# miguelmartin75/txt2vid

Measured on AMD Instinct MI355X. Metric: TGANv2 GAN train throughput (G+D steps x global batch), 16x64x64 videos/sec, higher is better.
Workload: dtype f32; 1 GPU; BASELINE configs[1]: unconditional TGANv2 16x64x64x1, per-GPU batch 32, fp32, RSGAN + GP 0.5, Adam 2e-4 (0.5,0.999), 1 D + 1 G step, subsample_input pyramid 8/16/32/64; global_batch=32, per_gpu_batch=32, parallelism=dp1

## Files before the change

### include/t2v_hip.h

```cpp
#ifndef T2V_HIP_H
#define T2V_HIP_H

#include <stdint.h>

#ifdef __cplusplus
extern "C" {
#endif

#define T2V_OK 0
#define T2V_EINVAL (-1)
#define T2V_ELAUNCH (-2)

#define T2V_MAX_TAPS 27

typedef struct {
    int32_t N, Cin, D, H, W, Cout;
    int32_t ntaps;
    int8_t dz[T2V_MAX_TAPS], dy[T2V_MAX_TAPS], dx[T2V_MAX_TAPS];
    int8_t pad_[3];
} t2v_conv_geom;

#define T2V_MAX_GROUPS 8
typedef struct {
    const float* x;
// ... 238 lines not shown

int t2v_copy2d(const float* src, int64_t src_ld, float* dst, int64_t dst_ld, int64_t rows, int64_t cols, void* stream);
int t2v_cast_bf16(const void* src, void* dst, int64_t n, int dir, void* stream);
int t2v_permute01(const float* x, float* y, int64_t A, int64_t B, int64_t inner, void* stream);
int t2v_permute12(const float* x, float* y, int64_t A, int64_t B, int64_t C, int64_t inner, void* stream);
int t2v_subsample_frames(float* x, float* y, int64_t b, int64_t T, int64_t inner, int64_t bo, int64_t To, int bt,
                         int adjoint, const int32_t* bt_dev , void* stream);
int t2v_pyramid_scatter(const float* g, float* gx, int B, int C, int T, int64_t HW, int Bo, int To, int sb, int st,
                        int bt, void* stream);


int t2v_scalar_combine(const void* const* ptrs, const float* weights, int n, float* out, void* stream);
int t2v_gather_rows(const float* x, const int32_t* perm, float* out, int64_t rows, int64_t cols, int inverse, void* stream);


typedef struct t2v_poolbox_job {
    const float* in;
    const float* mask;
    float* out;
    const float* bias;
    int32_t NC, D, H, W;
    int32_t tmode, relu;
    float scale;
    int32_t C;
} t2v_poolbox_job;
int t2v_pool_boxsum(const t2v_poolbox_job* jobs, int njobs, void* stream);
int t2v_pool_unbox(const t2v_poolbox_job* jobs, int njobs, void* stream);
int64_t t2v_pool_conv_fwd_ws_floats(const t2v_conv_group* groups, int ngroups, int Cin, int Cout);
int t2v_pool_conv_fwd(const t2v_conv_group* groups, int ngroups, int Cin, int Cout, const float* wp, const float* bias, float* ws,
                      int flags, void* stream);
// ... 59 lines not shown
```

### txt2vid_amd/_lib.py

```python
import ctypes as C
import os

_HERE = os.path.dirname(os.path.abspath(__file__))
LIB_PATH = os.environ.get('T2V_LIB') or os.path.join(_HERE, 'csrc', 'libt2v_hip.so')

MAX_TAPS = 27


class ConvGeom(C.Structure):
    _fields_ = [('N', C.c_int32), ('Cin', C.c_int32), ('D', C.c_int32), ('H', C.c_int32), ('W', C.c_int32),
                ('Cout', C.c_int32), ('ntaps', C.c_int32),
                ('dz', C.c_int8 * MAX_TAPS), ('dy', C.c_int8 * MAX_TAPS), ('dx', C.c_int8 * MAX_TAPS),
                ('pad_', C.c_int8 * 3)]


class ConvGroup(C.Structure):
    _fields_ = [('x', C.c_void_p), ('y', C.c_void_p), ('mask', C.c_void_p), ('N', C.c_int32), ('D', C.c_int32), ('H', C.c_int32), ('W', C.c_int32),
                ('ntaps', C.c_int32), ('dstride', C.c_int32), ('ydstride', C.c_int32), ('yoff', C.c_int32), ('Dy', C.c_int32),
                ('dz', C.c_int8 * MAX_TAPS), ('dy', C.c_int8 * MAX_TAPS), ('dx', C.c_int8 * MAX_TAPS), ('widx', C.c_int8 * MAX_TAPS)]


class AdamJob(C.Structure):
    _fields_ = [('p', C.c_void_p), ('g', C.c_void_p), ('m', C.c_void_p), ('v', C.c_void_p), ('n', C.c_int64)]

# ... 154 lines not shown
    't2v_adam_multi': [_P, _I, _F, _F, _F, _F, _F, _F, _F, _P, _P],
    't2v_sgd_multi': [_P, _I, _F, _F, _F, _I, _P],
    't2v_adam_tick': [_P, _F, _F, _P],
    't2v_ema_multi': [_P, _I, _F, _F, _P, _F, _P],
    't2v_ema_tick': [_P, _P],
    't2v_swap_multi': [_P, _I, _P],
    't2v_pyramid_gather': [_P, _P, _I, _I, _I, _I, _I, _I, _I, _I, _I, _I, _I, _I, _P, _P],
    't2v_copy2d': [_P, _L, _P, _L, _L, _L, _P],
    't2v_cast_bf16': [_P, _P, _L, _I, _P],
    't2v_permute01': [_P, _P, _L, _L, _L, _P],
    't2v_permute12': [_P, _P, _L, _L, _L, _L, _P],
    't2v_subsample_frames': [_P, _P, _L, _L, _L, _L, _L, _I, _I, _P, _P],
    't2v_pyramid_scatter': [_P, _P, _I, _I, _I, _L, _I, _I, _I, _I, _I, _P],
    't2v_scalar_combine': [_P, C.POINTER(C.c_float), _I, _P, _P],
    't2v_gather_rows': [_P, _P, _P, _L, _L, _I, _P],
    't2v_pool_boxsum': [_P, _I, _P],
    't2v_pool_unbox': [_P, _I, _P],
    't2v_pool_conv_fwd_ws_floats': [_P, _I, _I, _I],
    't2v_pool_conv_fwd': [_P, _I, _I, _I, _P, _P, _P, _I, _P],
    't2v_pool_conv_dgrad': [_P, _I, _I, _I, _P, _P],
    't2v_pool_conv_dgrad_splits': [_P, _I, _I, _I],
    't2v_pool_conv_wgrad_slab_floats': [_P, _I, _I, _I, _I, _I],
    't2v_pool_conv_wgrad': [_P, _I, _I, _I, _I, _P, _P, _P, _I, _P],
    't2v_pool_conv_wgrad_partial': [_P, _I, _I, _I, _I, _P, _I, _I, _P, _P],
    't2v_wgrad_swap': [_P, _P, _I, _I, _I, _I, _P],
    't2v_pool_conv_plan': [_I, _P, _I, _I, _I, _I3],
    't2v_synth_clips': [_P, _I, _L, _I, _I, _I, _I3, _P, _P, _P, _P],
    't2v_clip_gather': [_P, _L, _P, _I, _I, _I, _I, _I, _P, _P, _P, _P],
    't2v_tseed_fwd_bn': [_P, _P, _P, _P, _P, _P, _P, _P, _P, _P, _P, _I, _I, _I, _I, _I, _F, _F, _I, _P],
    't2v_tseed_fwd_tanh': [_P, _P, _P, _P, _P, _I, _I, _I, _I, _P],
# ... 39 lines not shown
```

### txt2vid_amd/csrc/conv.hip

```cpp
#include <hip/hip_runtime.h>
#include <stdint.h>
#include "../../include/t2v_hip.h"

typedef float f32x16 __attribute__((ext_vector_type(16)));

#ifdef T2V_STAMPS
__device__ unsigned long long* g_stamps = nullptr;
__device__ unsigned int g_stamps_cap = 0;
extern "C" int t2v_stamps_set(void* buf, unsigned int cap_records) {
    if (hipMemcpyToSymbol(HIP_SYMBOL(g_stamps), &buf, sizeof(buf)) != hipSuccess) return -1;
    if (hipMemcpyToSymbol(HIP_SYMBOL(g_stamps_cap), &cap_records, sizeof(cap_records)) != hipSuccess) return -1;
    return 0;
}
__device__ __forceinline__ unsigned long long stamp_now() {
    unsigned long long t;
    __builtin_amdgcn_sched_barrier(0);
    asm volatile("s_memtime %0\n\ts_waitcnt lgkmcnt(0)" : "=s"(t) :: "memory");
    __builtin_amdgcn_sched_barrier(0);
    return t;
}
#define STAMP(v) const unsigned long long v = stamp_now()
#define STAMP_ACC(acc, a, b) acc += (b) - (a)
#else
#define STAMP(v)
// ... 1081 lines not shown
    __shared__ __attribute__((aligned(16))) float Bs[(DB ? 2 : 1) * 3 * BKT * BN];

    const int tid = threadIdx.x;
    const int lane = tid & 63, wave = tid >> 6;
    const int l31 = lane & 31, hi = lane >> 5;
    const int wco = wave % WAVES_CO, wm = wave / WAVES_CO;

    const int tile = xcd_remap((int)blockIdx.x, (int)gridDim.x);
    int gi = 0;
#pragma unroll
    for (int k = 1; k < T2V_MAX_GROUPS; ++k)
        if (k < tab.n && tile >= tab.tile_start[k]) gi = k;
    const t2v_conv_group& gd = tab.g[gi];
    const int tm = gd.dstride;
    const int Dn = tm ? gd.D / 2 : 1, Hn = gd.H / 2, Wn = gd.W / 2;
    const int Hp = gd.H + 1, Wp = gd.W + 2, Dp = tm ? gd.D + 1 : 1;
    const int Vp = Dp * Hp * Wp;
    const int HWn = Hn * Wn, DHWn = Dn * HWn;
    const int M = gd.N * DHWn;
    const int m0 = (tile - tab.tile_start[gi]) * BM, co0 = blockIdx.y * BN;
    const int ntaps = gd.ntaps;
    const int nrow = ntaps / 3;

    const int lane_r = lane < nrow ? lane : 0, lane_t = lane < ntaps ? lane : 0;
    const int tab_roff = ((tm ? gd.dz[lane_r * 3] + 1 : 0) * Hp + gd.dy[lane_r * 3] + 1) * Wp * 4;
    const int tab_widx = gd.widx[lane_t];
    const __amdgpu_buffer_rsrc_t rx = __builtin_amdgcn_make_buffer_rsrc((void*)gd.x, 0, (int)((uint32_t)(gd.N * Vp) * (uint32_t)Cin * 4u), 0x00020000);
    const __amdgpu_buffer_rsrc_t rw = __builtin_amdgcn_make_buffer_rsrc((void*)wp, 0, -1, 0x00020000);

    const int ma_l = tid % BM, ka_l = tid / BM;
    uint32_t xbase = 0;
// ... 213 lines not shown
    const int wco = wave % WAVES_CO, wm = wave / WAVES_CO;

    const int tile = xcd_remap((int)blockIdx.x, (int)gridDim.x);
    int gi = 0;
#pragma unroll
    for (int k = 1; k < T2V_MAX_GROUPS; ++k)
        if (k < tab.n && tile >= tab.tile_start[k]) gi = k;
    const t2v_conv_group& gd = tab.g[gi];
    const int tm = gd.dstride;
    const int nct = (int)gridDim.y >> 2;
    const int pair = (int)blockIdx.y / nct, ct = pair >> 1, cy = pair & 1;
    if (tm == 0 && ct) return;
    const int co0 = ((int)blockIdx.y - pair * nct) * BN;
    const int Dn = tm ? gd.D / 2 : 1, Hn = gd.H / 2, Wn = gd.W / 2;
    const int Dq = tm ? Dn + 1 : 1, Hq = Hn + 1, Wq = Wn + 1;
    const int HWn = Hn * Wn, Vn = Dn * HWn;
    const int HWq = Hq * Wq, Vq = Dq * HWq;
    const int De = (tm && ct) ? Dn : Dq, He = cy ? Hn : Hq;
    const int HWe = He * Wq, Ve = De * HWe;
    const int M = gd.N * Ve;
    const int m0 = (tile - tab.tile_start[gi]) * BM;
    if (m0 >= M) return;
    const int ndz = (tm && ct == 0) ? 2 : 1, ndy = cy == 0 ? 2 : 1;
    const int nrow = ndz * ndy;
    const int lane_t = lane < 27 ? lane : 0;
    const int tab_widx = gd.widx[lane_t];
    const __amdgpu_buffer_rsrc_t rx = __builtin_amdgcn_make_buffer_rsrc((void*)gd.x, 0, (int)((uint32_t)(gd.N * Vn) * (uint32_t)K * 4u), 0x00020000);
    const __amdgpu_buffer_rsrc_t rw = __builtin_amdgcn_make_buffer_rsrc((void*)wp, 0, -1, 0x00020000);

    const int ma_l = tid % BM, ka_l = tid / BM;
    const int hk = tid % BKT;
    const bool halo_thread = tid < BKT;
// ... 217 lines not shown
                const float xo = a_own[krow * AP], xl = a_left[krow * AP];
                acc0 = __builtin_amdgcn_mfma_f32_32x32x2f32(b0[krow * BN], xo, acc0, 0, 0, 0);
                acc1 = __builtin_amdgcn_mfma_f32_32x32x2f32(b1[krow * BN], xo, acc1, 0, 0, 0);
                acc0 = __builtin_amdgcn_mfma_f32_32x32x2f32(b2[krow * BN], xl, acc0, 0, 0, 0);
            }
        }
        __builtin_amdgcn_s_setprio(0);
        __syncthreads();
    }
    }
    const int m = m0 + wm * WM + l31;
    if (m < M) {
        const int n = m / Ve, spe = m - n * Ve;
        const int at = spe / HWe, r2 = spe - at * HWe;
        const int a = r2 / Wq, b = r2 - a * Wq;
        const int sp = (at * Hq + a) * Wq + b;
        constexpr bool row_ok = true;
        const bool ok1 = b < Wn;
        const size_t plane = (size_t)gd.N * C * Vq;
        float* p0 = gd.y + ((size_t)blockIdx.z * 8 + (size_t)((ct * 2 + cy) * 2 + 0)) * plane + (size_t)n * C * Vq + sp;
        float* p1 = p0 + plane;
#pragma unroll
        for (int r = 0; r < 16; ++r) {
            const int co = co0 + wco * WCO + (r & 3) + 8 * (r >> 2) + 4 * hi;
            if (co < C) {
                if (row_ok) p0[(size_t)co * Vq] = acc0[r];
                if (ok1) p1[(size_t)co * Vq] = acc1[r];
            }
        }
    }
}
// ... 2208 lines not shown
#pragma unroll
        for (int k = 1; k < T2V_MAX_GROUPS; ++k)
            if (k < tab.n && q >= tab.chunk_start[k]) gi = k;
        const t2v_conv_group& gd = tab.g[gi];
        g_i = gi;
        g_begin = tab.chunk_start[gi];
        g_end = tab.chunk_start[gi + 1];
        g_tm = gd.dstride;
        const int Dn = g_tm ? gd.D / 2 : 1;
        gHn = gd.H / 2; gWn = gd.W / 2; gHWn = gHn * gWn; gVn = Dn * gHWn;
        gM = gd.N * gVn;
        g_pow2 = ((Dn & (Dn - 1)) | (gHn & (gHn - 1)) | (gWn & (gWn - 1))) == 0;
        g_lw = __builtin_ctz(gWn);
        g_lhw = g_lw + __builtin_ctz(gHn);
        g_lv = g_lhw + __builtin_ctz(Dn);
        gHp = gd.H + 1; gWp = gd.W + 2;
        gVp = (g_tm ? gd.D + 1 : 1) * gHp * gWp;
        g_x = __builtin_amdgcn_make_buffer_rsrc((void*)gd.x, 0, (int)((uint32_t)(gd.N * gVp) * (uint32_t)Cin * 4u), 0x00020000);
        g_y = __builtin_amdgcn_make_buffer_rsrc((void*)gd.y, 0, (int)((uint32_t)gM * (uint32_t)Cout * 4u), 0x00020000);
    };

    auto load_chunk = [&](int q) {
        if (q >= g_end || g_i < 0) enter_group(q);
        const int m = (q - g_begin) * WG_BK + ml;
        const bool mv = m < gM;
        int n, sp, e, i, j;
        if (g_pow2) {
            n = m >> g_lv;
            sp = m & (gVn - 1);
            e = sp >> g_lhw;
            i = (sp >> g_lw) & (gHn - 1);
// ... 550 lines not shown
    WGroupTable tab;
    WgradPlan p;
    if (!build_wtable(groups, ngroups, Cin, Cout, kD, kH, kW, false, tab, p)) return T2V_EINVAL;
    float dummy;
    return wgrad_impl(groups, ngroups, Cin, Cout, kD, kH, kW, nullptr, want_bias ? &dummy : nullptr, slab, flags, stream, out_src);
}
struct PoolPlan { int S; long tiles; bool vecb; };
static bool pool_member_ok(const t2v_conv_group& g, bool need_ptrs) {
    if (need_ptrs && (!g.x || !g.y)) return false;
    if (g.N < 1 || g.H < 2 || g.W < 2 || (g.H & 1) || (g.W & 1)) return false;
    if (g.dstride == 0) return g.D == 1;
    if (g.dstride != 1 && g.dstride != 2) return false;
    return g.D >= 2 && !(g.D & 1);
}
static inline long pool_rows(const t2v_conv_group& g) { return (long)g.N * (g.dstride ? g.D / 2 : 1) * (g.H / 2) * (g.W / 2); }
static inline long pool_padded(const t2v_conv_group& g) { return (long)(g.dstride ? g.D + 1 : 1) * (g.H + 1) * (g.W + 2); }
static inline long pool_grid(const t2v_conv_group& g) { return (long)(g.dstride ? g.D / 2 + 1 : 1) * (g.H / 2 + 1) * (g.W / 2 + 1); }

static bool build_pool_fwd(const t2v_conv_group* groups, int ngroups, int Cin, int Cout, bool need_ptrs, GroupTable& tab, PoolPlan& p) {
    if (!groups || ngroups < 1 || ngroups > T2V_MAX_GROUPS || Cin < 32 || (Cin % 32) || Cout < 4 || (Cout % 4)) return false;
    long mt = 0, ot = 0;
    int max_rows = 1;
    tab.n = ngroups;
    for (int i = 0; i < ngroups; ++i) {
        const t2v_conv_group& g = groups[i];
        if (!pool_member_ok(g, need_ptrs)) return false;
        if ((long)g.N * pool_padded(g) * Cin >= (1L << 29) || pool_rows(g) * Cout >= (1L << 31)) return false;
        if (g.ntaps != 9 && g.ntaps != 27) return false;
        if (g.dstride == 0 && g.ntaps != 9) return false;
        for (int r = 0; r < g.ntaps / 3; ++r)
            for (int d = 0; d < 3; ++d) {
// ... 69 lines not shown
        long blocks = (tab.out_start[ngroups] + 255) / 256;
        if (blocks > 2048) blocks = 2048;
        ProfScope prof_r(4, 0.0, s, Mtot, Cin, Cout, taps, ngroups, p.S);
        T2V_LAUNCH_PROF(splitk_reduce_kernel, dim3((unsigned)blocks), dim3(256), 0, s, tab, ws, bias, p.S, Cout, flags);
    }
    return launch_status();
}

static bool build_pool_dgrad(const t2v_conv_group* groups, int ngroups, int K, int C, bool need_ptrs, GroupTable& tab, PoolPlan& p) {
    if (!groups || ngroups < 1 || ngroups > T2V_MAX_GROUPS || K < 32 || (K % 32) || C < 4 || (C % 4)) return false;
    long mt = 0;
    tab.n = ngroups;
    for (int i = 0; i < ngroups; ++i) {
        const t2v_conv_group& g = groups[i];
        if (!pool_member_ok(g, need_ptrs)) return false;
        if (pool_rows(g) * K >= (1L << 29) || (long)g.N * pool_grid(g) * C * 8 >= (1L << 31)) return false;
        for (int f = 0; f < 27; ++f) {
            const bool live = g.dstride != 0 || (f / 9) == 1;
            if (live && (g.widx[f] < 0 || g.widx[f] >= T2V_MAX_TAPS)) return false;
        }
        tab.g[i] = g;
        tab.tile_start[i] = (int32_t)mt;
        tab.out_start[i] = 0;
        mt += ((long)g.N * pool_grid(g) + 63) / 64;
    }
    for (int i = ngroups; i <= T2V_MAX_GROUPS; ++i) { tab.tile_start[i] = (int32_t)mt; tab.out_start[i] = 0; }
    p.tiles = mt * 4 * ((C + 63) / 64);
    p.vecb = (C % 4) == 0;
    long S = 1;
    const long ncb = K / 32;
    static const long split_below = env_long("T2V_POOL_DGRAD_SPLIT_BELOW", 576);
// ... 487 lines not shown
```

### txt2vid_amd/csrc/pointwise.hip

```cpp
#include <hip/hip_runtime.h>
#include <stdint.h>
#include "../../include/t2v_hip.h"

#define T2V_LAUNCH(...) do { (void)hipGetLastError(); hipLaunchKernelGGL(__VA_ARGS__); } while (0)

static inline int launch_status() {
    hipError_t e = hipGetLastError();
    return e == hipSuccess ? T2V_OK : -(int)e - 1000;
}
static inline unsigned nblocks(long n, int per = 256) {
    long b = (n + per - 1) / per;
    if (b > 2048) b = 2048;
    if (b < 1) b = 1;
    return (unsigned)b;
}
#define GRID_STRIDE(i, n) for (long i = (long)blockIdx.x * blockDim.x + threadIdx.x; i < (n); i += (long)gridDim.x * blockDim.x)
#define S_(stream) ((hipStream_t)(stream))

__device__ __forceinline__ float wave_sum(float v) {
#pragma unroll
    for (int o = 32; o > 0; o >>= 1) v += __shfl_xor(v, o, 64);
    return v;
}
__device__ __forceinline__ float wave_max(float v) {
// ... 2650 lines not shown
    T2V_LAUNCH(gather_rows_k, dim3(nblocks(rows * cols)), dim3(256), 0, S_(st), x, perm, out, (long)rows, (long)cols, inverse);
    return launch_status();
}

extern "C" const char* t2v_version(void) { return "t2v_hip 0.1 (gfx950, fp32 MFMA)"; }

struct PoolBoxBatch { t2v_poolbox_job j[POOL_MT]; int begin[POOL_MT + 1]; int n; };

__device__ __forceinline__ uint32_t small_div(uint32_t m, uint32_t d, float rcp) {
    int q = (int)((float)m * rcp);
    const int r = (int)m - q * (int)d;
    q += (r >= (int)d) ? 1 : 0;
    q -= (r < 0) ? 1 : 0;
    return (uint32_t)q;
}
__global__ __launch_bounds__(256) void pool_boxsum_k(const PoolBoxBatch tb) {
    int ji = 0;
#pragma unroll
    for (int k = 1; k < POOL_MT; ++k)
        if (k < tb.n && (int)blockIdx.x >= tb.begin[k]) ji = k;
    const t2v_poolbox_job& q = tb.j[ji];
    const int D = q.D, H = q.H, W = q.W, tm = q.tmode;
    const uint32_t Dp = tm ? D + 1 : 1, Hp = H + 1, Wp = W + 2, Wp2 = Wp / 2;
    const uint32_t n2 = (uint32_t)q.NC * Dp * Hp * Wp2;
    const uint32_t base = (uint32_t)((int)blockIdx.x - tb.begin[ji]) * POOL_CHUNK;
    const uint32_t b_r0 = base / Wp2, b_x = base - b_r0 * Wp2;
    const uint32_t b_r1 = b_r0 / Hp, b_y = b_r0 - b_r1 * Hp;
    const uint32_t b_nc = b_r1 / Dp, b_f = b_r1 - b_nc * Dp;
    const float rW = 1.0f / (float)Wp2, rH = 1.0f / (float)Hp, rD = 1.0f / (float)Dp;
    const float* __restrict__ x = q.in;
    const float* __restrict__ mk = q.mask;
    const float floor_ = q.relu ? 0.f : -__builtin_inff();
    const float scale = q.scale;
    const int nf = tm == 1 ? 2 : 1;
    float2* __restrict__ out2 = reinterpret_cast<float2*>(q.out);
#pragma unroll
    for (int it = 0; it < POOL_CHUNK / 256; ++it) {
        const uint32_t t = it * 256 + threadIdx.x;
// ... 22 lines not shown
                if (y0 && c1) v01 = mk[o + 1] > 0.f ? v01 : 0.f;
                if (y0 && c2) v02 = mk[o + 2] > 0.f ? v02 : 0.f;
                if (y1 && c0) v10 = mk[o + W] > 0.f ? v10 : 0.f;
                if (y1 && c1) v11 = mk[o + W + 1] > 0.f ? v11 : 0.f;
                if (y1 && c2) v12 = mk[o + W + 2] > 0.f ? v12 : 0.f;
            }
            v00 = fmaxf(v00, floor_); v01 = fmaxf(v01, floor_); v02 = fmaxf(v02, floor_);
            v10 = fmaxf(v10, floor_); v11 = fmaxf(v11, floor_); v12 = fmaxf(v12, floor_);
            a0 += (v00 + v01) + (v10 + v11);
            a1 += (v01 + v02) + (v11 + v12);
        }
        out2[base + t] = make_float2(a0 * scale, xp + 1 <= (uint32_t)W ? a1 * scale : 0.f);
    }
}

__global__ __launch_bounds__(256) void pool_unbox_k(const PoolBoxBatch tb) {
    int ji = 0;
#pragma unroll
    for (int k = 1; k < POOL_MT; ++k)
        if (k < tb.n && (int)blockIdx.x >= tb.begin[k]) ji = k;
    const t2v_poolbox_job& q = tb.j[ji];
    const uint32_t D = q.D, H = q.H, W = q.W, W2 = W / 2;
    const int tm = q.tmode;
    const uint32_t Dq = tm ? D / 2 + 1 : 1, Hq = H / 2 + 1, Wq = W / 2 + 1;
    const uint32_t n2 = (uint32_t)q.NC * D * H * W2;
    const uint32_t plane = (uint32_t)q.NC * Dq * Hq * Wq;
    const int sets = q.relu > 1 ? q.relu : 1;
    const uint32_t base = (uint32_t)((int)blockIdx.x - tb.begin[ji]) * POOL_CHUNK;
    const uint32_t b_r0 = base / W2, b_x = base - b_r0 * W2;
    const uint32_t b_r1 = b_r0 / H, b_y = b_r0 - b_r1 * H;
    const uint32_t b_nc = b_r1 / D, b_f = b_r1 - b_nc * D;
    const float rW = 1.0f / (float)W2, rH = 1.0f / (float)H, rD = 1.0f / (float)D;
    const float* __restrict__ pl = q.in;
    const float2* __restrict__ mk2 = reinterpret_cast<const float2*>(q.mask);
    float2* __restrict__ out2 = reinterpret_cast<float2*>(q.out);
    const int nf = tm == 1 ? 2 : 1;
#pragma unroll
    for (int it = 0; it < POOL_CHUNK / 256; ++it) {
        const uint32_t t = it * 256 + threadIdx.x;
// ... 16 lines not shown
                    const uint32_t o1 = o0 + plane;
                    for (int s_ = 0; s_ < sets; ++s_) {
                        const uint32_t so = (uint32_t)s_ * 8u * plane;
                        const float e0 = pl[o0 + so], e1 = pl[o0 + 1 + so], d1 = pl[o1 + so];
                        a0 += e0 + d1;
                        a1 += e1 + d1;
                    }
                }
            }
        }
        const float bv = q.bias ? q.bias[nc % (uint32_t)q.C] : 0.f;
        out2[base + t] = make_float2(m2.x > 0.f ? a0 * q.scale + bv : 0.f, m2.y > 0.f ? a1 * q.scale + bv : 0.f);
    }
}

static int poolbox_multi(const t2v_poolbox_job* jobs, int njobs, bool unbox, void* st) {
    if (!jobs || njobs < 1) return T2V_EINVAL;
    for (int at = 0; at < njobs; at += POOL_MT) {
        PoolBoxBatch tb;
        const int cnt = njobs - at < POOL_MT ? njobs - at : POOL_MT;
        long blocks = 0;
        for (int i = 0; i < cnt; ++i) {
            const t2v_poolbox_job& q = jobs[at + i];
            if (!q.in || !q.out || q.NC < 1 || q.D < 1 || q.H < 2 || q.W < 2 || (q.H & 1) || (q.W & 1) || q.tmode < 0 || q.tmode > 2) return T2V_EINVAL;
            if ((q.tmode == 0 && q.D != 1) || (q.tmode != 0 && (q.D < 2 || (q.D & 1)))) return T2V_EINVAL;
            if (q.bias && (!unbox || q.C < 1 || (q.NC % q.C) != 0)) return T2V_EINVAL;
            tb.j[i] = q;
            tb.begin[i] = (int)blocks;
            const long n = unbox ? (long)q.NC * q.D * q.H * q.W
                                 : (long)q.NC * (q.tmode ? q.D + 1 : 1) * (q.H + 1) * (q.W + 2);
            const long sets = unbox && q.relu > 1 ? q.relu : 1;
            if (n >= (1L << 31) || (unbox && 8 * sets * (long)q.NC * (q.tmode ? q.D / 2 + 1 : 1) * (q.H / 2 + 1) * (q.W / 2 + 1) >= (1L << 31)))
                return T2V_EINVAL;
            if (((uintptr_t)q.out & 7u) || (unbox && q.mask && ((uintptr_t)q.mask & 7u))) return T2V_EINVAL;
            blocks += (n / 2 + POOL_CHUNK - 1) / POOL_CHUNK;
        }
        for (int i = cnt; i <= POOL_MT; ++i) tb.begin[i] = (int)blocks;
        for (int i = cnt; i < POOL_MT; ++i) tb.j[i] = tb.j[0];
        tb.n = cnt;
        if (blocks > 0x7fffffffL) return T2V_EINVAL;
        if (unbox) T2V_LAUNCH(pool_unbox_k, dim3((unsigned)blocks), dim3(256), 0, S_(st), tb);
        else T2V_LAUNCH(pool_boxsum_k, dim3((unsigned)blocks), dim3(256), 0, S_(st), tb);
    }
    return launch_status();
}
extern "C" int t2v_pool_boxsum(const t2v_poolbox_job* jobs, int njobs, void* st) { return poolbox_multi(jobs, njobs, false, st); }
extern "C" int t2v_pool_unbox(const t2v_poolbox_job* jobs, int njobs, void* st) { return poolbox_multi(jobs, njobs, true, st); }

__global__ __launch_bounds__(256) void wgrad_swap_k(const float* __restrict__ src, float* __restrict__ dst, int Cout, int Cin, int T, int accum) {
    const long n = (long)Cout * Cin * T;
    GRID_STRIDE(i, n) {
        const int t = (int)(i % T); const long r = i / T;
        const int ci = (int)(r % Cin), co = (int)(r / Cin);
        const float v = src[((long)ci * Cout + co) * T + (T - 1 - t)];
        dst[i] = accum ? dst[i] + v : v;
    }
}
// ... 79 lines not shown
```

### txt2vid_amd/functional_pool.py

```python
import ctypes as C
import os

import torch
from torch.autograd import Function
from torch.autograd.function import once_differentiable

from ._lib import lib, check, ConvGroup, PoolBoxJob, WgradSrc, MAX_GROUPS
from ._ops import _stream, _p, _c

_DISABLED = os.environ.get('T2V_NO_POOLCONV') is not None
_NO_UPCONV = os.environ.get('T2V_NO_UPCONV') is not None


def _TF():
    from . import functional
    return functional


def pool_tmode(shape, stem):
    D, H, W = shape[2], shape[3], shape[4]
    if H < 2 or W < 2 or H % 2 or W % 2:
        return None
    if D == 1:
        return 0
# ... 3 lines not shown


def pool_scale(tmode):
    return 0.125 if tmode == 1 else 0.25


def pool_conv_ok(xs, w, stem):
    TF = _TF()
    if _DISABLED or TF.CONV_PRECISION != 'fp32' or not (1 <= len(xs) <= MAX_GROUPS) or w.dim() != 5 or tuple(w.shape[2:]) != (3, 3, 3):
        return False
    if w.shape[0] % 32 or w.shape[1] % 32 or not xs[0].is_cuda:
        return False
    return all(x.dim() == 5 and pool_tmode(x.shape, stem) is not None for x in xs)


def pooled_shape(shape, tmode):
    N, _, D, H, W = shape
    return (N, D // 2 if tmode else 1, H // 2, W // 2)



def _box_jobs(ins, masks, outs, shapes, tmodes, relu, scale=None, bias=None):
    arr = (PoolBoxJob * len(ins))()
    for a, t, sh, tm, i in zip(arr, ins, shapes, tmodes, range(len(ins))):
        a.in_, a.out = t.data_ptr(), outs[i].data_ptr()
        a.mask = masks[i].data_ptr() if masks is not None else None
        a.bias = bias.data_ptr() if bias is not None else None
        a.NC, a.D, a.H, a.W, a.C = sh[0] * sh[1], sh[2], sh[3], sh[4], sh[1]
        a.tmode, a.relu, a.scale = tm, int(relu), pool_scale(tm) if scale is None else scale
    return arr


def boxsum_raw(ins, tmodes, relu, masks=None, scale=None):
    ins = [_c(t) for t in ins]
    masks = [_c(m) for m in masks] if masks is not None else None
    shapes = [tuple(t.shape) for t in ins]
    outs = [torch.empty((sh[0], sh[1], sh[2] + 1 if tm else 1, sh[3] + 1, sh[4] + 2), device=t.device, dtype=torch.float32)
            for t, sh, tm in zip(ins, shapes, tmodes)]
    check(lib().t2v_pool_boxsum(_box_jobs(ins, masks, outs, shapes, tmodes, relu, scale), len(ins), _stream()), 't2v_pool_boxsum')
    return outs


def unbox_raw(planes, shapes, tmodes, masks=None, scale=None, bias=None):
    masks = [_c(m) for m in masks] if masks is not None else None
    outs = [torch.empty(tuple(sh), device=p.device, dtype=torch.float32) for p, sh in zip(planes, shapes)]
    sets = planes[0].shape[0] if planes[0].dim() == 7 else 1
    check(lib().t2v_pool_unbox(_box_jobs(planes, masks, outs, shapes, tmodes, sets, scale, bias), len(planes), _stream()), 't2v_pool_unbox')
    return outs


def _tap_union(tmodes, kD=3):
    TF = _TF()
# ... 54 lines not shown
    cout, cin = (w5.shape[1], w5.shape[0]) if transpose else (w5.shape[0], w5.shape[1])
    ts = _tap_union(tmodes, w5.shape[2])
    slot_of = {t: j for j, t in enumerate(ts.taps)}
    arr = (ConvGroup * len(gzs))()
    for a, g, sh, tm in zip(arr, gzs, shapes, tmodes):
        if tuple(g.shape) != (sh[0], cout) + pooled_shape(sh, tm)[1:]:
            raise ValueError('pooled gradient of shape %s for a member of shape %s' % (tuple(g.shape), tuple(sh)))
        a.x, a.y, a.mask = g.data_ptr(), None, None
        a.N, a.D, a.H, a.W = sh[0], sh[2], sh[3], sh[4]
        a.dstride, a.ntaps = tm, 27
        for f in range(27):
            a.widx[f] = slot_of.get(26 - f, -1) if ts.T == 27 else (slot_of.get(8 - (f - 9), -1) if 9 <= f < 18 else -1)
    S = int(lib().t2v_pool_conv_dgrad_splits(arr, len(gzs), cout, cin))
    if S < 1:
        raise RuntimeError('bad pooled data-gradient geometry')
    planes = [torch.empty((S, 8, sh[0], cin, sh[2] // 2 + 1 if tm else 1, sh[3] // 2 + 1, sh[4] // 2 + 1), device=g.device, dtype=torch.float32)
              for g, sh, tm in zip(gzs, shapes, tmodes)]
    for a, pl in zip(arr, planes):
        a.y = pl.data_ptr()
    wp = TF.packed_weight(w5, ts, 0 if transpose else 1)
    check(lib().t2v_pool_conv_dgrad(arr, len(gzs), cout, cin, _p(wp), _stream()), 't2v_pool_conv_dgrad')
    return planes


def _wgrad_table(rts, gzs, shapes, tmodes):
    arr = (ConvGroup * len(rts))()
    for a, x, g, sh, tm in zip(arr, rts, gzs, shapes, tmodes):
        a.x, a.y, a.mask = x.data_ptr(), g.data_ptr(), None
        a.N, a.D, a.H, a.W = sh[0], sh[2], sh[3], sh[4]
        a.dstride, a.ntaps = tm, 27 if tm else 9
    return arr
# ... 218 lines not shown
```

Baseline: 3008 videos/s.

## Pad pooled box-sum planes to 4-float pitch and add vectorized box/unbox kernels

Pads the innermost row extent of the box-sum and pooled data-gradient planes to a multiple of four floats, and updates the conv forward, dgrad and wgrad indexing plus the host allocations to use the new pitch. New box-sum and unbox kernels each handle four or eight outputs per thread with 128-bit buffer loads and stores. The old pair kernels stay as a fallback when widths or alignment do not fit. This is meant to cut memory-instruction count in the pooling stages, at the cost of slightly larger buffers and padded columns that must stay consistent across all consumers.

```diff
diff --git a/include/t2v_hip.h b/include/t2v_hip.h
--- a/include/t2v_hip.h
+++ b/include/t2v_hip.h
@@ -276,6 +276,8 @@
 int t2v_gather_rows(const float* x, const int32_t* perm, float* out, int64_t rows, int64_t cols, int inverse, void* stream);
 
 
+#define T2V_POOL_PITCH(n) (((n) + 3) & ~3)
+int t2v_pool_pitch(int n);
 typedef struct t2v_poolbox_job {
     const float* in;
     const float* mask;
diff --git a/txt2vid_amd/_lib.py b/txt2vid_amd/_lib.py
--- a/txt2vid_amd/_lib.py
+++ b/txt2vid_amd/_lib.py
@@ -192,6 +192,7 @@
     't2v_pyramid_scatter': [_P, _P, _I, _I, _I, _L, _I, _I, _I, _I, _I, _P],
     't2v_scalar_combine': [_P, C.POINTER(C.c_float), _I, _P, _P],
     't2v_gather_rows': [_P, _P, _P, _L, _L, _I, _P],
+    't2v_pool_pitch': [_I],
     't2v_pool_boxsum': [_P, _I, _P],
     't2v_pool_unbox': [_P, _I, _P],
     't2v_pool_conv_fwd_ws_floats': [_P, _I, _I, _I],
diff --git a/txt2vid_amd/csrc/conv.hip b/txt2vid_amd/csrc/conv.hip
--- a/txt2vid_amd/csrc/conv.hip
+++ b/txt2vid_amd/csrc/conv.hip
@@ -1119,7 +1119,7 @@
     const t2v_conv_group& gd = tab.g[gi];
     const int tm = gd.dstride;
     const int Dn = tm ? gd.D / 2 : 1, Hn = gd.H / 2, Wn = gd.W / 2;
-    const int Hp = gd.H + 1, Wp = gd.W + 2, Dp = tm ? gd.D + 1 : 1;
+    const int Hp = gd.H + 1, Wp = T2V_POOL_PITCH(gd.W + 2), Dp = tm ? gd.D + 1 : 1;
     const int Vp = Dp * Hp * Wp;
     const int HWn = Hn * Wn, DHWn = Dn * HWn;
     const int M = gd.N * DHWn;
@@ -1363,8 +1363,9 @@
     const int co0 = ((int)blockIdx.y - pair * nct) * BN;
     const int Dn = tm ? gd.D / 2 : 1, Hn = gd.H / 2, Wn = gd.W / 2;
     const int Dq = tm ? Dn + 1 : 1, Hq = Hn + 1, Wq = Wn + 1;
+    const int Pq = T2V_POOL_PITCH(Wq);
     const int HWn = Hn * Wn, Vn = Dn * HWn;
-    const int HWq = Hq * Wq, Vq = Dq * HWq;
+    const int Vq = Dq * Hq * Pq;
     const int De = (tm && ct) ? Dn : Dq, He = cy ? Hn : Hq;
     const int HWe = He * Wq, Ve = De * HWe;
     const int M = gd.N * Ve;
@@ -1612,7 +1613,7 @@
         const int n = m / Ve, spe = m - n * Ve;
         const int at = spe / HWe, r2 = spe - at * HWe;
         const int a = r2 / Wq, b = r2 - a * Wq;
-        const int sp = (at * Hq + a) * Wq + b;
+        const int sp = (at * Hq + a) * Pq + b;
         constexpr bool row_ok = true;
         const bool ok1 = b < Wn;
         const size_t plane = (size_t)gd.N * C * Vq;
@@ -3851,7 +3852,7 @@
         g_lw = __builtin_ctz(gWn);
         g_lhw = g_lw + __builtin_ctz(gHn);
         g_lv = g_lhw + __builtin_ctz(Dn);
-        gHp = gd.H + 1; gWp = gd.W + 2;
+        gHp = gd.H + 1; gWp = T2V_POOL_PITCH(gd.W + 2);
         gVp = (g_tm ? gd.D + 1 : 1) * gHp * gWp;
         g_x = __builtin_amdgcn_make_buffer_rsrc((void*)gd.x, 0, (int)((uint32_t)(gd.N * gVp) * (uint32_t)Cin * 4u), 0x00020000);
         g_y = __builtin_amdgcn_make_buffer_rsrc((void*)gd.y, 0, (int)((uint32_t)gM * (uint32_t)Cout * 4u), 0x00020000);
@@ -4432,7 +4433,8 @@
     return g.D >= 2 && !(g.D & 1);
 }
 static inline long pool_rows(const t2v_conv_group& g) { return (long)g.N * (g.dstride ? g.D / 2 : 1) * (g.H / 2) * (g.W / 2); }
-static inline long pool_padded(const t2v_conv_group& g) { return (long)(g.dstride ? g.D + 1 : 1) * (g.H + 1) * (g.W + 2); }
+static inline long pool_padded(const t2v_conv_group& g) { return (long)(g.dstride ? g.D + 1 : 1) * (g.H + 1) * T2V_POOL_PITCH(g.W + 2); }
+static inline long pool_plane(const t2v_conv_group& g) { return (long)(g.dstride ? g.D / 2 + 1 : 1) * (g.H / 2 + 1) * T2V_POOL_PITCH(g.W / 2 + 1); }
 static inline long pool_grid(const t2v_conv_group& g) { return (long)(g.dstride ? g.D / 2 + 1 : 1) * (g.H / 2 + 1) * (g.W / 2 + 1); }
 
 static bool build_pool_fwd(const t2v_conv_group* groups, int ngroups, int Cin, int Cout, bool need_ptrs, GroupTable& tab, PoolPlan& p) {
@@ -4532,7 +4534,7 @@
     for (int i = 0; i < ngroups; ++i) {
         const t2v_conv_group& g = groups[i];
         if (!pool_member_ok(g, need_ptrs)) return false;
-        if (pool_rows(g) * K >= (1L << 29) || (long)g.N * pool_grid(g) * C * 8 >= (1L << 31)) return false;
+        if (pool_rows(g) * K >= (1L << 29) || (long)g.N * pool_plane(g) * C * 8 >= (1L << 31)) return false;
         for (int f = 0; f < 27; ++f) {
             const bool live = g.dstride != 0 || (f / 9) == 1;
             if (live && (g.widx[f] < 0 || g.widx[f] >= T2V_MAX_TAPS)) return false;
diff --git a/txt2vid_amd/csrc/pointwise.hip b/txt2vid_amd/csrc/pointwise.hip
--- a/txt2vid_amd/csrc/pointwise.hip
+++ b/txt2vid_amd/csrc/pointwise.hip
@@ -2688,14 +2688,14 @@
     q -= (r < 0) ? 1 : 0;
     return (uint32_t)q;
 }
-__global__ __launch_bounds__(256) void pool_boxsum_k(const PoolBoxBatch tb) {
+__global__ __launch_bounds__(256) void pool_boxsum_pair_k(const PoolBoxBatch tb) {
     int ji = 0;
 #pragma unroll
     for (int k = 1; k < POOL_MT; ++k)
         if (k < tb.n && (int)blockIdx.x >= tb.begin[k]) ji = k;
     const t2v_poolbox_job& q = tb.j[ji];
     const int D = q.D, H = q.H, W = q.W, tm = q.tmode;
-    const uint32_t Dp = tm ? D + 1 : 1, Hp = H + 1, Wp = W + 2, Wp2 = Wp / 2;
+    const uint32_t Dp = tm ? D + 1 : 1, Hp = H + 1, Wp = T2V_POOL_PITCH(W + 2), Wp2 = Wp / 2;
     const uint32_t n2 = (uint32_t)q.NC * Dp * Hp * Wp2;
     const uint32_t base = (uint32_t)((int)blockIdx.x - tb.begin[ji]) * POOL_CHUNK;
     const uint32_t b_r0 = base / Wp2, b_x = base - b_r0 * Wp2;
@@ -2748,7 +2748,7 @@
     }
 }
 
-__global__ __launch_bounds__(256) void pool_unbox_k(const PoolBoxBatch tb) {
+__global__ __launch_bounds__(256) void pool_unbox_pair_k(const PoolBoxBatch tb) {
     int ji = 0;
 #pragma unroll
     for (int k = 1; k < POOL_MT; ++k)
@@ -2756,7 +2756,7 @@
     const t2v_poolbox_job& q = tb.j[ji];
     const uint32_t D = q.D, H = q.H, W = q.W, W2 = W / 2;
     const int tm = q.tmode;
-    const uint32_t Dq = tm ? D / 2 + 1 : 1, Hq = H / 2 + 1, Wq = W / 2 + 1;
+    const uint32_t Dq = tm ? D / 2 + 1 : 1, Hq = H / 2 + 1, Wq = T2V_POOL_PITCH(W / 2 + 1);
     const uint32_t n2 = (uint32_t)q.NC * D * H * W2;
     const uint32_t plane = (uint32_t)q.NC * Dq * Hq * Wq;
     const int sets = q.relu > 1 ? q.relu : 1;
@@ -2803,12 +2803,164 @@
     }
 }
 
+#define POOL_WIDE 256
+typedef uint32_t pool_u32x4 __attribute__((ext_vector_type(4)));
+__device__ __forceinline__ __amdgpu_buffer_rsrc_t pool_rsrc(const void* p, uint32_t bytes) {
+    return __builtin_amdgcn_make_buffer_rsrc(const_cast<void*>(p), 0, (int)bytes, 0x00020000);
+}
+__device__ __forceinline__ float4 pool_ld4(__amdgpu_buffer_rsrc_t r, uint32_t off, bool ok, uint32_t bytes) {
+    return __builtin_bit_cast(float4, __builtin_amdgcn_raw_buffer_load_b128(r, ok ? off : bytes, 0, 0));
+}
+__device__ __forceinline__ float pool_ld1(__amdgpu_buffer_rsrc_t r, uint32_t off, bool ok, uint32_t bytes) {
+    return __builtin_bit_cast(float, __builtin_amdgcn_raw_buffer_load_b32(r, ok ? off : bytes, 0, 0));
+}
+__device__ __forceinline__ void pool_st4(__amdgpu_buffer_rsrc_t r, uint32_t off, float4 v) {
+    __builtin_amdgcn_raw_buffer_store_b128(__builtin_bit_cast(pool_u32x4, v), r, off, 0, 0);
+}
+
+__global__ __launch_bounds__(256) void pool_boxsum_k(const PoolBoxBatch tb) {
+    int ji = 0;
+#pragma unroll
+    for (int k = 1; k < POOL_MT; ++k)
+        if (k < tb.n && (int)blockIdx.x >= tb.begin[k]) ji = k;
+    const t2v_poolbox_job& q = tb.j[ji];
+    const int D = q.D, H = q.H, W = q.W, tm = q.tmode;
+    const uint32_t Dp = tm ? D + 1 : 1, Hp = H + 1, P4 = T2V_POOL_PITCH(W + 2) / 4;
+    const uint32_t n4 = (uint32_t)q.NC * Dp * Hp * P4;
+    const uint32_t base = (uint32_t)((int)blockIdx.x - tb.begin[ji]) * POOL_WIDE;
+    const uint32_t t = threadIdx.x;
+    if (base + t >= n4) return;
+    const uint32_t b_r0 = base / P4, b_x = base - b_r0 * P4;
+    const uint32_t b_r1 = b_r0 / Hp, b_y = b_r0 - b_r1 * Hp;
+    const uint32_t b_nc = b_r1 / Dp, b_f = b_r1 - b_nc * Dp;
+    const float rW = 1.0f / (float)P4, rH = 1.0f / (float)Hp, rD = 1.0f / (float)Dp;
+    const uint32_t ix = b_x + t, q1 = small_div(ix, P4, rW), xq = (ix - q1 * P4) * 4;
+    const uint32_t iy = b_y + q1, q2 = small_div(iy, Hp, rH), yp = iy - q2 * Hp;
+    const uint32_t if_ = b_f + q2, q3 = small_div(if_, Dp, rD), fp = if_ - q3 * Dp;
+    const uint32_t nc = b_nc + q3;
+    const uint32_t in_bytes = (uint32_t)q.NC * D * H * W * 4u;
+    const __amdgpu_buffer_rsrc_t rin = pool_rsrc(q.in, in_bytes);
+    const __amdgpu_buffer_rsrc_t rmk = pool_rsrc(q.mask ? q.mask : q.in, in_bytes);
+    const __amdgpu_buffer_rsrc_t rout = pool_rsrc(q.out, n4 * 16u);
+    const bool has_mask = q.mask != nullptr;
+    const float floor_ = q.relu ? 0.f : -__builtin_inff();
+    const float scale = q.scale;
+    const int nf = tm == 1 ? 2 : 1;
+    const int f0 = tm == 0 ? 0 : (int)fp - 1;
+    const bool y0 = yp >= 1, y1 = yp < (uint32_t)H;
+    const bool cq = xq < (uint32_t)W, cl = xq >= 1;
+    float a0 = 0.f, a1 = 0.f, a2 = 0.f, a3 = 0.f;
+    for (int a = 0; a < nf; ++a) {
+        const int f = f0 + a;
+        if ((unsigned)f >= (unsigned)D) continue;
+        const uint32_t o = (((nc * D + f) * H + (yp - 1)) * W + xq) * 4u;
+        const uint32_t o1 = o + (uint32_t)W * 4u;
+        float4 u = pool_ld4(rin, o, y0 && cq, in_bytes), v = pool_ld4(rin, o1, y1 && cq, in_bytes);
+        float ul = pool_ld1(rin, o - 4u, y0 && cl, in_bytes), vl = pool_ld1(rin, o1 - 4u, y1 && cl, in_bytes);
+        if (has_mask) {
+            const float4 mu = pool_ld4(rmk, o, y0 && cq, in_bytes), mv = pool_ld4(rmk, o1, y1 && cq, in_bytes);
+            const float mul = pool_ld1(rmk, o - 4u, y0 && cl, in_bytes), mvl = pool_ld1(rmk, o1 - 4u, y1 && cl, in_bytes);
+            u.x = mu.x > 0.f ? u.x : 0.f; u.y = mu.y > 0.f ? u.y : 0.f; u.z = mu.z > 0.f ? u.z : 0.f; u.w = mu.w > 0.f ? u.w : 0.f;
+            v.x = mv.x > 0.f ? v.x : 0.f; v.y = mv.y > 0.f ? v.y : 0.f; v.z = mv.z > 0.f ? v.z : 0.f; v.w = mv.w > 0.f ? v.w : 0.f;
+            ul = mul > 0.f ? ul : 0.f;
+            vl = mvl > 0.f ? vl : 0.f;
+        }
+        ul = fmaxf(ul, floor_); u.x = fmaxf(u.x, floor_); u.y = fmaxf(u.y, floor_); u.z = fmaxf(u.z, floor_); u.w = fmaxf(u.w, floor_);
+        vl = fmaxf(vl, floor_); v.x = fmaxf(v.x, floor_); v.y = fmaxf(v.y, floor_); v.z = fmaxf(v.z, floor_); v.w = fmaxf(v.w, floor_);
+        a0 += (ul + u.x) + (vl + v.x);
+        a1 += (u.x + u.y) + (v.x + v.y);
+        a2 += (u.y + u.z) + (v.y + v.z);
+        a3 += (u.z + u.w) + (v.z + v.w);
+    }
+    pool_st4(rout, (base + t) * 16u, make_float4(a0 * scale, cq ? a1 * scale : 0.f, cq ? a2 * scale : 0.f, cq ? a3 * scale : 0.f));
+}
+
+__global__ __launch_bounds__(256) void pool_unbox_k(const PoolBoxBatch tb) {
+    int ji = 0;
+#pragma unroll
+    for (int k = 1; k < POOL_MT; ++k)
+        if (k < tb.n && (int)blockIdx.x >= tb.begin[k]) ji = k;
+    const t2v_poolbox_job& q = tb.j[ji];
+    const uint32_t D = q.D, H = q.H, W = q.W, W8 = (W + 7) / 8;
+    const int tm = q.tmode;
+    const uint32_t Dq = tm ? D / 2 + 1 : 1, Hq = H / 2 + 1, Pq = T2V_POOL_PITCH(W / 2 + 1);
+    const uint32_t n8 = (uint32_t)q.NC * D * H * W8;
+    const uint32_t plane = (uint32_t)q.NC * Dq * Hq * Pq;
+    const int sets = q.relu > 1 ? q.relu : 1;
+    const uint32_t base = (uint32_t)((int)blockIdx.x - tb.begin[ji]) * POOL_WIDE;
+    const uint32_t t = threadIdx.x;
+    if (base + t >= n8) return;
+    const uint32_t b_r0 = base / W8, b_x = base - b_r0 * W8;
+    const uint32_t b_r1 = b_r0 / H, b_y = b_r0 - b_r1 * H;
+    const uint32_t b_nc = b_r1 / D, b_f = b_r1 - b_nc * D;
+    const float rW = 1.0f / (float)W8, rH = 1.0f / (float)H, rD = 1.0f / (float)D;
+    const uint32_t ix = b_x + t, q1 = small_div(ix, W8, rW), j = ix - q1 * W8;
+    const uint32_t iy = b_y + q1, q2 = small_div(iy, H, rH), y = iy - q2 * H;
+    const uint32_t if_ = b_f + q2, q3 = small_div(if_, D, rD), f = if_ - q3 * D;
+    const uint32_t nc = b_nc + q3;
+    const uint32_t out_bytes = (uint32_t)q.NC * D * H * W * 4u, pl_bytes = (uint32_t)sets * 8u * plane * 4u;
+    const __amdgpu_buffer_rsrc_t rpl = pool_rsrc(q.in, pl_bytes);
+    const __amdgpu_buffer_rsrc_t rmk = pool_rsrc(q.mask ? q.mask : q.in, q.mask ? out_bytes : 0u);
+    const __amdgpu_buffer_rsrc_t rout = pool_rsrc(q.out, out_bytes);
+    const bool hi4 = 8 * j + 4 < W;
+    const uint32_t oo = ((((nc * D + f) * H + y) * W) + 8 * j) * 4u;
+    float4 ma = make_float4(1.f, 1.f, 1.f, 1.f), mb = ma;
+    if (q.mask) {
+        ma = pool_ld4(rmk, oo, true, out_bytes);
+        mb = pool_ld4(rmk, oo + 16u, hi4, out_bytes);
+    }
+    float a0 = 0.f, a1 = 0.f, a2 = 0.f, a3 = 0.f, a4 = 0.f, a5 = 0.f, a6 = 0.f, a7 = 0.f;
+    const int nf = tm == 1 ? 2 : 1;
+    for (int a = 0; a < nf; ++a) {
+        const uint32_t pt = tm == 0 ? 0u : f + 1 - a;
+        const uint32_t ct = pt & 1u, at = pt >> 1;
+#pragma unroll
+        for (int b = 0; b < 2; ++b) {
+            const uint32_t py = y + 1 - b, cy = py & 1u, ay = py >> 1;
+            const uint32_t o0 = (((ct * 2 + cy) * 2 + 0) * plane + ((nc * Dq + at) * Hq + ay) * Pq + 4 * j) * 4u;
+            const uint32_t o1 = o0 + plane * 4u;
+            for (int s_ = 0; s_ < sets; ++s_) {
+                const uint32_t so = (uint32_t)s_ * 8u * plane * 4u;
+                const float4 e = pool_ld4(rpl, o0 + so, true, pl_bytes), d = pool_ld4(rpl, o1 + so, true, pl_bytes);
+                const float e4 = pool_ld1(rpl, o0 + so + 16u, hi4, pl_bytes);
+                a0 += e.x + d.x;
+                a1 += e.y + d.x;
+                a2 += e.y + d.y;
+                a3 += e.z + d.y;
+                a4 += e.z + d.z;
+                a5 += e.w + d.z;
+                a6 += e.w + d.w;
+                a7 += e4 + d.w;
+            }
+        }
+    }
+    const float bv = q.bias ? q.bias[nc % (uint32_t)q.C] : 0.f;
+    const float sc = q.scale;
+    pool_st4(rout, oo, make_float4(ma.x > 0.f ? a0 * sc + bv : 0.f, ma.y > 0.f ? a1 * sc + bv : 0.f,
+                                   ma.z > 0.f ? a2 * sc + bv : 0.f, ma.w > 0.f ? a3 * sc + bv : 0.f));
+    if (hi4)
+        pool_st4(rout, oo + 16u, make_float4(mb.x > 0.f ? a4 * sc + bv : 0.f, mb.y > 0.f ? a5 * sc + bv : 0.f,
+                                             mb.z > 0.f ? a6 * sc + bv : 0.f, mb.w > 0.f ? a7 * sc + bv : 0.f));
+}
+
+extern "C" int t2v_pool_pitch(int n) { return n < 1 ? T2V_EINVAL : T2V_POOL_PITCH(n); }
+
 static int poolbox_multi(const t2v_poolbox_job* jobs, int njobs, bool unbox, void* st) {
     if (!jobs || njobs < 1) return T2V_EINVAL;
     for (int at = 0; at < njobs; at += POOL_MT) {
         PoolBoxBatch tb;
         const int cnt = njobs - at < POOL_MT ? njobs - at : POOL_MT;
         long blocks = 0;
+        bool wide = true;
+        for (int i = 0; i < cnt; ++i) {
+            const t2v_poolbox_job& q = jobs[at + i];
+            if (q.W < 4 || (q.W & 3) || q.NC < 1 || q.D < 1 || q.H < 2) { wide = false; continue; }
+            const long full = (long)q.NC * q.D * q.H * q.W;
+            const long rt = (long)q.NC * (q.tmode ? q.D + 1 : 1) * (q.H + 1) * T2V_POOL_PITCH(q.W + 2);
+            const long pl = 8L * (q.relu > 1 ? q.relu : 1) * q.NC * (q.tmode ? q.D / 2 + 1 : 1) * (q.H / 2 + 1) * T2V_POOL_PITCH(q.W / 2 + 1);
+            if (full >= (1L << 30) || (unbox ? pl : rt) >= (1L << 30)) wide = false;
+            if ((((uintptr_t)q.in | (uintptr_t)q.out | (uintptr_t)q.mask) & 15u)) wide = false;
+        }
         for (int i = 0; i < cnt; ++i) {
             const t2v_poolbox_job& q = jobs[at + i];
             if (!q.in || !q.out || q.NC < 1 || q.D < 1 || q.H < 2 || q.W < 2 || (q.H & 1) || (q.W & 1) || q.tmode < 0 || q.tmode > 2) return T2V_EINVAL;
@@ -2817,19 +2969,27 @@
             tb.j[i] = q;
             tb.begin[i] = (int)blocks;
             const long n = unbox ? (long)q.NC * q.D * q.H * q.W
-                                 : (long)q.NC * (q.tmode ? q.D + 1 : 1) * (q.H + 1) * (q.W + 2);
+                                 : (long)q.NC * (q.tmode ? q.D + 1 : 1) * (q.H + 1) * T2V_POOL_PITCH(q.W + 2);
             const long sets = unbox && q.relu > 1 ? q.relu : 1;
-            if (n >= (1L << 31) || (unbox && 8 * sets * (long)q.NC * (q.tmode ? q.D / 2 + 1 : 1) * (q.H / 2 + 1) * (q.W / 2 + 1) >= (1L << 31)))
+            if (n >= (1L << 31) ||
+                (unbox && 8 * sets * (long)q.NC * (q.tmode ? q.D / 2 + 1 : 1) * (q.H / 2 + 1) * T2V_POOL_PITCH(q.W / 2 + 1) >= (1L << 31)))
                 return T2V_EINVAL;
             if (((uintptr_t)q.out & 7u) || (unbox && q.mask && ((uintptr_t)q.mask & 7u))) return T2V_EINVAL;
-            blocks += (n / 2 + POOL_CHUNK - 1) / POOL_CHUNK;
+            if (wide) {
+                const long groups = unbox ? (long)q.NC * q.D * q.H * ((q.W + 7) / 8) : n / 4;
+                blocks += (groups + POOL_WIDE - 1) / POOL_WIDE;
+            } else {
+                blocks += (n / 2 + POOL_CHUNK - 1) / POOL_CHUNK;
+            }
         }
         for (int i = cnt; i <= POOL_MT; ++i) tb.begin[i] = (int)blocks;
         for (int i = cnt; i < POOL_MT; ++i) tb.j[i] = tb.j[0];
         tb.n = cnt;
         if (blocks > 0x7fffffffL) return T2V_EINVAL;
-        if (unbox) T2V_LAUNCH(pool_unbox_k, dim3((unsigned)blocks), dim3(256), 0, S_(st), tb);
-        else T2V_LAUNCH(pool_boxsum_k, dim3((unsigned)blocks), dim3(256), 0, S_(st), tb);
+        if (unbox && wide) T2V_LAUNCH(pool_unbox_k, dim3((unsigned)blocks), dim3(256), 0, S_(st), tb);
+        else if (unbox) T2V_LAUNCH(pool_unbox_pair_k, dim3((unsigned)blocks), dim3(256), 0, S_(st), tb);
+        else if (wide) T2V_LAUNCH(pool_boxsum_k, dim3((unsigned)blocks), dim3(256), 0, S_(st), tb);
+        else T2V_LAUNCH(pool_boxsum_pair_k, dim3((unsigned)blocks), dim3(256), 0, S_(st), tb);
     }
     return launch_status();
 }
diff --git a/txt2vid_amd/functional_pool.py b/txt2vid_amd/functional_pool.py
--- a/txt2vid_amd/functional_pool.py
+++ b/txt2vid_amd/functional_pool.py
@@ -41,6 +41,18 @@
     return all(x.dim() == 5 and pool_tmode(x.shape, stem) is not None for x in xs)
 
 
+_pitch = {}
+
+
+def pool_pitch(n):
+    p = _pitch.get(n)
+    if p is None:
+        p = _pitch[n] = int(lib().t2v_pool_pitch(n))
+        if p < n:
+            raise RuntimeError('bad pooled row extent %d' % n)
+    return p
+
+
 def pooled_shape(shape, tmode):
     N, _, D, H, W = shape
     return (N, D // 2 if tmode else 1, H // 2, W // 2)
@@ -62,7 +74,7 @@
     ins = [_c(t) for t in ins]
     masks = [_c(m) for m in masks] if masks is not None else None
     shapes = [tuple(t.shape) for t in ins]
-    outs = [torch.empty((sh[0], sh[1], sh[2] + 1 if tm else 1, sh[3] + 1, sh[4] + 2), device=t.device, dtype=torch.float32)
+    outs = [torch.empty((sh[0], sh[1], sh[2] + 1 if tm else 1, sh[3] + 1, pool_pitch(sh[4] + 2)), device=t.device, dtype=torch.float32)
             for t, sh, tm in zip(ins, shapes, tmodes)]
     check(lib().t2v_pool_boxsum(_box_jobs(ins, masks, outs, shapes, tmodes, relu, scale), len(ins), _stream()), 't2v_pool_boxsum')
     return outs
@@ -147,7 +159,7 @@
     S = int(lib().t2v_pool_conv_dgrad_splits(arr, len(gzs), cout, cin))
     if S < 1:
         raise RuntimeError('bad pooled data-gradient geometry')
-    planes = [torch.empty((S, 8, sh[0], cin, sh[2] // 2 + 1 if tm else 1, sh[3] // 2 + 1, sh[4] // 2 + 1), device=g.device, dtype=torch.float32)
+    planes = [torch.empty((S, 8, sh[0], cin, sh[2] // 2 + 1 if tm else 1, sh[3] // 2 + 1, pool_pitch(sh[4] // 2 + 1)), device=g.device, dtype=torch.float32)
               for g, sh, tm in zip(gzs, shapes, tmodes)]
     for a, pl in zip(arr, planes):
         a.y = pl.data_ptr()
```

Result: no change. 3014 videos/s, median of 6 (+0.2%).
